# youzhenfei1995/DistributedTF

Measured on AMD Instinct MI355X. Metric: images/sec (whole node) ResNet-56 CIFAR-10 PBT pop=8 at 1/2/4/8 MI355X, higher is better.
Workload: dtype bf16; 1 GPU; model=resnet56_v2_cifar, global_batch=1024, per_member_batch=128, population=8, parallelism=pbt_pop8_8members_per_gpu, backend=hip, exploit_every=25, step_graph=captured

## Files before the change

distributedtf_amd/engine/hip_resnet.py:

```python

from __future__ import annotations

import ctypes
import os
from typing import List, Sequence, Tuple

import torch

from .. import ops
from ..data.datasets import IndexBatch, batch_len
from ..models.resnet import BN_EPS
from .hip_step import (HipBackend, HipPlan, LossRing, PinnedStager, _LIVE_GRAPH_PLANS, _p, advance_steps,
                       graph_state, note_step_advanced, release_graphs, run_captured, run_optimizer, same_batches,
                       upload_hyper)

def _nrep() -> int:
    return ops.build_nrep()


DET_WG_PER_MEMBER = 64
SMALL_POP_MAX = 2
FWD_ITERS_PER_WG = int(os.environ.get("DTF_FWD_ITERS", "4"))
FWD_ITERS_C = {64: 2}
FWD_WG_TARGET = {16: int(os.environ.get("DTF_FWD_WG16", "512"))}
# ... 375 lines not shown
        return p.loss_view()


class _StepPlan(HipPlan):

    def __init__(self, be: HipResNetBackend, slots: List[int], sizes: List[int], src=None, eval_mode=False,
                 elastic_cap=None):
        self.elastic = bool(elastic_cap) and not eval_mode
        self.real_sizes = list(sizes)
        if self.elastic:
            sizes = [int(elastic_cap)] * len(slots)
        self._init_members(be, slots, sizes, eval_mode, counts=self.real_sizes)
        e, dev, N = be.e, be.dev, self.N
        L = be.L
        prog = L.prog
        cfg = L.cfg
        self._wgen, self._elastic_red = [], {}
        self._grab = None
        self._cnt_stage = self._rng_stage = None
        self._stamp_n, self.stamp_rows = {"fwd": 0, "fused": 0}, []
        self._det_rows = self.slab_buf = None
        self._slot_index = {}
        self.uniform = (len(set(sizes)) == 1 and list(slots) == list(range(len(slots))) and not self.elastic
                        and not be.det)
        if self.elastic:
            self.first_t = torch.tensor([self.first[s] for s in slots], dtype=torch.int32, device=dev)
        self.ring = LossRing(len(slots), dev) if (dev.type == "cuda" and not eval_mode and len(slots) <= 1024) else None
        H = cfg.image_size
        self.x_in = torch.zeros(N, H, H, 3, dtype=torch.float32, device=dev)
        self.labels = torch.zeros(N, dtype=torch.int32, device=dev)
        self.xin16 = torch.zeros(N, H, H, 16, dtype=ops.act_dtype(), device=dev)
        self.src = src
        if src is not None:
            self.idx = torch.zeros(N, dtype=torch.long, device=dev)
            self.rng = torch.zeros(2, dtype=torch.int32, device=dev)
        self.v1 = cfg.version == 1
        self.xs, self.hs, self.scs = [], [], []
        self.hb = []
        self.h0 = torch.empty(N, H, H, cfg.num_filters, dtype=ops.act_dtype(), device=dev) if self.v1 else None
        pool = {}

        def act(kind, hw_, c_, i_=0):
            if not self.eval:
                return torch.empty(N, hw_, hw_, c_, dtype=ops.act_dtype(), device=dev)
            key = (kind, hw_, c_, i_ % 2 if kind == "x" else 0)
            if key not in pool:
                pool[key] = torch.empty(N, hw_, hw_, c_, dtype=ops.act_dtype(), device=dev)
            return pool[key]

        hw, c = H, cfg.num_filters
        self.xs.append(act("x", hw, c, 0))
        for bi, blk in enumerate(prog.blocks):
            ca = prog.convs[blk.convs[0]]
            hw_o = hw // blk.stride
            self.hs.append(act("h", hw_o, ca.cout))
            self.scs.append(act("sc", hw_o, ca.cout) if blk.proj is not None else None)
            self.xs.append(act("x", hw_o, ca.cout, bi + 1))
            if self.v1:
                self.hb.append(act("hb", hw_o, ca.cout))
            hw = hw_o
        self._work_cache, self._uniform_geo = {}, {}
        self._pending_slab = None
        if self.eval:
            nb = len(prog.bns)
            cap = e.capacity
            self.ev_stats = torch.zeros(nb, cap, be.nrep, 128, dtype=torch.float32, device=dev)
            self.ev_sink = torch.zeros(cap, be.nrep, 128, dtype=torch.float32, device=dev)
            self.ev_acc = torch.zeros(2, cap, dtype=torch.float32, device=dev)
            self.logits = None
            self._build_eval()
            return
        self.tmp = {}
        hw, c = H, cfg.num_filters
        for st in range(len(cfg.block_sizes)):
            if st > 0:
                hw //= 2
            cc = cfg.num_filters * (2 ** st)
            self.tmp[hw] = dict(g=[torch.empty(N, hw, hw, cc, dtype=ops.act_dtype(), device=dev) for _ in range(2)],
                                dz2=torch.empty(N, hw, hw, cc, dtype=ops.act_dtype(), device=dev),
                                dz1=torch.empty(N, hw, hw, cc, dtype=ops.act_dtype(), device=dev))
        self.pd = {}
        hw = H
        for blk in prog.blocks:
            if blk.proj is not None:
                ci = prog.convs[blk.proj].cin
                self.pd[id(blk)] = torch.empty(N, hw, hw, ci, dtype=ops.act_dtype(), device=dev)
            hw //= blk.stride
        self.dfeat = torch.zeros(N, cfg.final_size, dtype=torch.float32, device=dev)
        v2gpu = dev.type == "cuda" and cfg.version == 2
        self.small_pop = v2gpu and len(slots) <= SMALL_POP_MAX and not be.det
        large = DEFER_MID_CS if (len(slots) <= DEFER_MID_POP and not be.det) else DEFER_LARGE_CS
        self.defer_cs = {16, 32, 64} if self.small_pop else (set(large) if v2gpu else set())
        self._wg_jobs = {}
        self._slab_flip = 0
        self._deferred = []
        self.wslab = dev.type == "cuda"
        self._deferred_dense = []
        self._build()
        assert self._pending_slab is None and not self._deferred and not self._deferred_dense, \
            "every dW slab must be reduced before the optimizer"
        if self.elastic:
            self._work_gen_launch()

    def _work_iters(self, bands, n_wg, det_per=None):
        det = self.be.det
        dper = (det_per or DET_WG_PER_MEMBER) if det else None
        key = ("it", bands, ("det", dper) if det else n_wg)
        w = self._work_cache.get(key)
        if w is None and self.elastic:
            per = dper if det else max(1, n_wg // max(1, len(self.slots)))
            w = self._elastic_table(per, bands, 1)
            self._work_cache[key] = w
        if w is None:
            items = []
            per_member = dper if det else max(1, n_wg // max(1, len(self.slots)))
            for s, n in zip(self.slots, self.sizes):
                total = n * bands
                f = self.first[s] * bands
                chunk = max(1, -(-total // per_member))
                for i in range(0, total, chunk):
                    items.append([f + i, min(chunk, total - i), 0, s])
                if det:
                    items += [[f, 0, 0, s]] * (per_member - -(-total // chunk))
                geo = (-(-total // chunk), chunk, total)
            w = torch.tensor(items, dtype=torch.int32, device=self.be.dev)
            self._work_cache[key] = w
            self._uniform_geo[w.data_ptr()] = geo
        return w

    def _set_uniform(self, a, work):
        if self.uniform:
            a.u_items, a.u_chunk, a.u_per = self._uniform_geo[work.data_ptr()]
            assert a.u_items * len(self.slots) == work.shape[0]

    def _elastic_table(self, per, bands, min_chunk, split=False):
        rows = 2 if split else 1
        host = []
        prop = int(ELASTIC_PROP and not self.be.det)
        layout = elastic_rows([n * bands for n in self.real_sizes], per, min_chunk, prop)
        for (s, n), (r0, nrows, chunk) in zip(zip(self.slots, self.real_sizes), layout):
            total, f = n * bands, self.first[s] * bands
            for j in range(nrows):
                st = j * chunk
                nit = min(chunk, total - st) if st < total else 0
                for z in range(rows):
                    host.append([f + st if nit > 0 else f, nit, z, s])
        assert len(host) == per * len(self.slots) * rows
        w = torch.tensor(host, dtype=torch.int32, device=self.be.dev)
        self._wgen.append((w, per, bands, min_chunk, int(split), prop))
        return w

    def _work_gen_launch(self):
        descs = (WorkGenDesc * len(self._wgen))()
        red = self._elastic_red
        for i, (w, per, bands, mc, sp, prop) in enumerate(self._wgen):
            descs[i] = WorkGenDesc(w.data_ptr(), _p(red.get(w.data_ptr())), per, bands, mc, sp, prop, 0)
        dt = torch.frombuffer(bytearray(bytes(descs)), dtype=torch.uint8).to(self.be.dev)
        self._hold(dt)
        self.launches.insert(0, (ops.lib().dtf_work_gen, (_p(dt), len(self._wgen), _p(self.slots_t),
                                                          _p(self.first_t), len(self.slots), _p(self.cnt))))

    def set_sizes(self, sizes):
        assert self.elastic and len(sizes) == len(self.slots) and max(sizes) <= self.sizes[0]
        if list(sizes) == self.real_sizes:
            return
        self.real_sizes = list(sizes)
        vals = [0.0] * self.e.capacity
# ... 37 lines not shown
        if w is None:
            per_member = max(1, target_items // max(1, len(self.slots)))
            w = self._chunks(lambda n: max(min_chunk, -(-n // per_member)))
            self._work_cache[key] = w
        return w

    def _base_args(self):
        be, e = self.be, self.e
        a = ConvArgs()
        a.img_slot = _p(self.img_slot)
        a.params = _p(e.state)
        a.p_mstride = e.S
        a.cnt = _p(self.cnt)
        a.w_mstride = be.L.wtot
        a.grads = _p(e.grads)
        a.g_mstride = e.Pp
        a.cin_real = 0
        return a

    def _bn(self, idx):
        b = self.be.L.prog.bns[idx]
        return b.gamma_off, b.beta_off

    def _add(self, fn, *args):
        if self._grab is not None:
            self._grab.append((fn, args))
            return
        super()._add(fn, *args)

    def _conv_fwd(self, ci, x, y, stats_bn, in_bn, res=None, proj=None):
        be, L = self.be, self.be.L
        c = L.prog.convs[ci]
        Hi = x.shape[1]
        Ho = Hi // c.stride
        cin = 16 if ci == L.prog.stem else c.cin
        P = (c.k - 1) // 2
        rows = None
        for r in range(min(8, Ho), 0, -1):
            rows_in = (r - 1) * c.stride + c.k
            if Ho % r == 0 and (r * Ho) % 16 == 0 and rows_in * (Hi + 2 * P) * (cin // 8) <= 4 * 256:
                rows = r
                break
        assert rows is not None, ("no valid band for conv", ci)
        s1 = c.k == 3 and c.stride == 1 and cin == c.cout and Hi == 512 // cin and stats_bn is not None
        if s1 and cin == 64 and self.N <= HALF_BANDS_MAX_IMGS and in_bn is not None and not be.det:
            rows = 4
        bands = Ho // rows
        lo = FWD_MIN_WG_SMALL if len(self.slots) <= SMALL_POP_MAX else FWD_MIN_WG
        iters = FWD_ITERS_C.get(cin, FWD_ITERS_PER_WG)
        if cin in FWD_WG_TARGET:
            iters = max(iters, min(8, self.N * bands // FWD_WG_TARGET[cin]))
        n_wg = self._n_wg_iters(self.N * bands, per_wg=iters, lo=lo, hi=max(1024, self.N * bands // iters))
        work = self._work_iters(bands, n_wg)
        a = self._base_args()
        a.x, a.y, a.res = _p(x), _p(y), _p(res)
        a.w, a.w_off = _p(be.wf), L.fwd_off[ci]
        a.work = _p(work)
        if in_bn is not None:
            a.in_gamma, a.in_beta = self._bn(in_bn)
            a.st_in = _p(self._st_r(in_bn))
        if stats_bn is not None:
            a.st_out = _p(self._st_w(stats_bn))
        a.Hi, a.Wi, a.Ho, a.Wo, a.rows = Hi, Hi, Ho, Ho, rows
        if proj is not None:
            cp = L.prog.convs[proj[0]]
            assert (cp.k, cp.stride, cp.cin, cp.cout) == (1, c.stride, c.cin, c.cout) and c.k == 3, (ci, proj[0])
            assert proj[1].shape == y.shape and in_bn is not None and res is None
            a.y2, a.w2_off = _p(proj[1]), L.fwd_off[proj[0]]
        rows_in = (rows - 1) * c.stride + c.k
        tsz = (rows_in * (Hi + 2 * P) * max(_cpad(cin), _cpad_fwd(cin)) + 8 + 63) // 64 * 64
        lds = 1280 + 2 * tsz * 2
        mode = 0 if in_bn is None else 1
        lib = ops.lib()
        if s1 and (rows == 8 or (rows == 4 and cin == 64)):
            self._set_uniform(a, work)
            a.cin_real = self._stamp_row("fwd", "fwd_s1 C=%d in=%d res=%d" % (cin, mode, res is not None))
            lds = 1280 + 2 * ((rows_in * _wpitch(cin) * _cpad_fwd(cin) + 8 + 63) // 64 * 64) * 2
            self._add(lib.dtf_conv_fwd_s1, ctypes.byref(a), cin, mode, int(res is not None), rows, work.shape[0], lds)
        else:
            self._add(lib.dtf_conv_fwd, ctypes.byref(a), cin, c.cout, c.stride, c.k, mode, int(res is not None),
                      int(stats_bn is not None), work.shape[0], lds)
        self._hold(a)

    def _conv_dgrad(self, ci, dy, y, Hi, mode, epi, dy2=None, in_bn=None, res=None, xm=None, ep_bn=None):
        be, L = self.be, self.be.L
        c = L.prog.convs[ci]
        S, K = c.stride, c.k
        Ho = Hi // S
        rows = None
        for r in range(min(8, Hi), 0, -1):
            rows_t = r + K - 1 if S == 1 else (r + K + S - 2) // S + 1
            if Hi % r == 0 and (r * Hi) % 16 == 0 and rows_t * (Ho + 2) * (c.cout // 8) <= 4 * 256:
                rows = r
                break
        assert rows is not None, ("no valid band for dgrad", ci)
        if S == 2 and K == 3:
            assert rows == 8 and Hi == 512 // c.cin, ("stride-2 dgrad geometry", ci, Hi, c.cin, rows)
        rows_t = rows + K - 1 if S == 1 else (rows + K + S - 2) // S + 1
        bands = Hi // rows
        n_wg = self._n_wg_iters(self.N * bands)
        work = self._work_iters(bands, n_wg)
        a = self._base_args()
        a.x, a.x2, a.y, a.res, a.xm = _p(dy), _p(dy2), _p(y), _p(res), _p(xm)
        a.w, a.w_off = _p(be.wd), L.dgr_off[ci]
        a.work = _p(work)
        if in_bn is not None:
            a.in_gamma, a.in_beta = self._bn(in_bn)
            a.st_in, a.st_in_b = _p(be.st_f(in_bn)), _p(be.st_b(in_bn))
        if ep_bn is not None:
            a.ep_gamma, a.ep_beta = self._bn(ep_bn)
            a.st_ep = _p(be.st_f(ep_bn))
            a.st_out = _p(be.st_b(ep_bn))
        a.Hi, a.Wi, a.Ho, a.Wo, a.rows = Hi, Hi, Ho, Ho, rows
        tsz = (rows_t * (Ho + 2) * _cpad(c.cout) + 63) // 64 * 64
        lds = 2304 + 2 * tsz * 2
        lib = ops.lib()
        self._add(lib.dtf_conv_dgrad, ctypes.byref(a), c.cin, c.cout, S, K, mode, epi, work.shape[0], lds)
        self._hold(a)

    @staticmethod
    def _trans_multi(ca_spec):
        return ca_spec.stride == 2 and ca_spec.k == 3 and (ca_spec.cin, ca_spec.cout) in ((16, 32), (32, 64))

    def _add_trans_multi(self, grabbed, ca_spec):
        (f_c, args_c), (f_a, args_a), (f_b, args_b) = grabbed
        lib = ops.lib()
        assert [ops.launcher_name(f) for f in (f_c, f_a, f_b)] == ["dtf_conv_wgrad", "dtf_conv_dgrad", "dtf_conv_wgrad"]
        assert args_c[1:6] == (ca_spec.cin, ca_spec.cout, 2, 3, 1) and args_c[6] == 2
        assert args_a[1:7] == (ca_spec.cin, ca_spec.cout, 2, 1, 0, 0)
        assert args_b[1:7] == (ca_spec.cin, ca_spec.cout, 2, 1, 1, 0)
        ac, aa, ab = args_c[0]._obj, args_a[0]._obj, args_b[0]._obj
        ac.n_main, aa.n_main, ab.n_main = args_c[7], args_a[7], args_b[7]
        nblocks = args_c[7] + args_a[7] + args_b[7]
        lds = max(args_c[8], args_a[8], args_b[8])
        self._add(lib.dtf_conv_trans_multi, ctypes.byref(ac), ctypes.byref(aa), ctypes.byref(ab), ca_spec.cin,
                  ca_spec.cout, nblocks, lds)

    def _conv_wgrad(self, ci, x, dy, mode_x, mode_dy, x_bn=None, dy_bn=None, dy2=None, cin_real=None):
        be, L, e = self.be, self.be.L, self.e
        c = L.prog.convs[ci]
        Hi = x.shape[1]
        Ho = Hi // c.stride
        cin = 16 if ci == L.prog.stem else c.cin
        P = (c.k - 1) // 2
        rows = None
        for r in range(min(8, Ho), 0, -1):
            if Ho % r or (r * Ho) % 32:
                continue
            rows_in = (r - 1) * c.stride + c.k
            if rows_in * (Hi + 2 * P) * (cin // 8) <= 4 * 256 and r * Ho * (c.cout // 8) <= 2 * 256:
                rows = r
                break
        if rows is None:
            rows = _pick_rows(Ho, Ho, 1, 32, target_items=1, max_rows=8)
        wn = c.cout * c.k * c.k * c.cin
        n_wg = max(64, min(WGRAD_WG_PER_MEMBER * len(self.slots), int(12e6 / (4.0 * wn))))
        if self.be.det and not self.wslab:
            n_wg = len(self.slots)
        work = self._work_iters(Ho // rows, n_wg)
        a = self._base_args()
        a.x, a.dy, a.dy2 = _p(x), _p(dy), _p(dy2)
        a.work = _p(work)
        a.g_off = c.off
        a.cin_real = c.cin if cin_real is None else cin_real
        if x_bn is not None:
            a.x_gamma, a.x_beta = self._bn(x_bn)
            a.st_x = _p(be.st_f(x_bn))
        if dy_bn is not None:
            a.in_gamma, a.in_beta = self._bn(dy_bn)
            a.st_in, a.st_in_b = _p(be.st_f(dy_bn)), _p(be.st_b(dy_bn))
        a.Hi, a.Wi, a.Ho, a.Wo, a.rows = Hi, Hi, Ho, Ho, rows
        rows_in = (rows - 1) * c.stride + c.k
        assert 32 % Ho == 0, "wgrad k-step addressing needs Wo | 32"
        xt = (rows_in * (Hi + 2 * P) * _cpad(cin) + 63) // 64 * 64
        dt = (rows * Ho * _cpad(c.cout) + 63) // 64 * 64
        lds = 1536 + 2 * (xt + dt) * 2
        lib = ops.lib()
        if self.wslab:
            kel = c.cout * c.k * c.k * a.cin_real
            a.slab = _p(self._layer_slab(work.shape[0] * kel))
            self._deferred_dense.append((a.slab, self._slab_table(work), c.off, kel))
        self._add(lib.dtf_conv_wgrad, ctypes.byref(a), cin, c.cout, c.stride, c.k, mode_x, mode_dy, work.shape[0], lds)
        self._hold(a)

    def _conv_bwd_fused(self, ci, dy, dz_out, x, mode_dy, dy2=None, dy_bn=None, x_bn=None, res=None, ident_x=False,
                        dy3=None, dy_out=None, chain_bn=None, chain_h=None):
        be, L = self.be, self.be.L
        c = L.prog.convs[ci]
        assert c.stride == 1 and c.k == 3 and c.cin == c.cout
        assert (mode_dy == 3) == (dy3 is not None)
        C, H = c.cin, x.shape[1]
        rows = None
        for r in (8, 4, 2):
            if H % r == 0 and (r * H) % 32 == 0 and (r + 2) * (H + 2) * (C // 8) <= 4 * 256:
                rows = r
                break
        assert rows == 8 and H == 512 // C and x.shape[2] == H, (C, H, rows)
        for t in (dy, dy2, dy3, dy_out, dz_out, x, res):
            assert t is None or tuple(t.shape) == (self.N, H, H, C), (t.shape, C, H)
        bands = H // rows
        if C in self.defer_cs:
            assert chain_bn is None, "chain_bn needs the fused launch (the deferred path is v2-only)"
            return self._conv_bwd_deferred(ci, rows, dy, dz_out, x, mode_dy, dy2, dy_bn, x_bn, res, ident_x, dy3,
                                           dy_out)
        n_wg = self._fused_nwg(C, bands, mode_dy)
        work = self._work_iters(bands, n_wg)
        a = self._bwd_args(ci, work, rows, dy, dy2, dy3, x, dy_bn, None if ident_x else x_bn,
                           dgrad=(dz_out, res, dy_out))
        if chain_bn is not None:
            assert ident_x and mode_dy == 2 and tuple(chain_h.shape) == (self.N, H, H, C)
            a.x3 = _p(chain_h)
            a.ep_gamma, a.ep_beta = self._bn(chain_bn)
            a.st_ep = _p(self._st_r(chain_bn))
            a.st_out = _p(be.st_b(chain_bn))
        tsz = ((rows + 2) * _wpitch(C) * _cpad(C) + 8 + 63) // 64 * 64
        raw = C >= 64
        nbuf = 4
        lds = 2304 + (nbuf * tsz + (2 * rows * H * _cpad(C) if raw else 0)) * 2
        if C == 16 and _lib_knob("dtf_fused16_wlds"):
# ... 231 lines not shown
        if self.eval:
            self._add(lib.dtf_bn_eval_stats, _p(e.state), e.S, 3 * e.Pp, _p(be.bn_table_t), len(L.bn_table),
                      _p(self.ev_stats), be.stats_bn_stride, _p(self.slots_t), nslots, _p(self.cnt))
        if self.src is not None:
            self._add("augment", None)
        else:
            self._add(lib.dtf_prep_input, _p(self.x_in), _p(self.xin16), self.N * L.cfg.image_size ** 2, 3)

    def _step_epilogue(self):
        be, e, L = self.be, self.e, self.be.L
        self._flush_slab()
        self._flush_deferred()
        self._add(ops.lib().dtf_bn_step_end, _p(e.state), e.S, 3 * e.Pp, _p(be.bn_table_t), len(L.bn_table),
                  _p(be.stats[0]), _p(be.stats[1]), be.stats_bn_stride, _p(self.slots_t), len(self.slots),
                  _p(self.cnt), _p(e.grads), e.Pp)
        self._add("optim", None)
        self._add("step", None)

    def _head_args(self, train):
        be, e, L = self.be, self.e, self.be.L
        prog, cfg = L.prog, L.cfg
        hwork = self._head_work() if train else self._work_member(target_items=HEAD_ITEMS)
        ha = self._hold(HeadArgs())
        ha.x, ha.labels, ha.work = _p(self.xs[-1]), _p(self.labels), _p(hwork)
        ha.params, ha.p_mstride = _p(e.state), e.S
        ha.gamma_off, ha.beta_off = (-1, -1) if self.v1 else self._bn(prog.final_bn)
        ha.dw_off, ha.db_off = prog.dense_w_off, prog.dense_b_off
        ha.g_mstride, ha.cnt = e.Pp, _p(self.cnt)
        ha.hw, ha.C, ha.ncls, ha.train = L.final_hw, cfg.final_size, cfg.num_classes, int(train)
        if train:
            st = (be.stats, be.stats) if self.v1 else (be.st_f(prog.final_bn), be.st_b(prog.final_bn))
            ha.st_f, ha.st_b, ha.grads = _p(st[0]), _p(st[1]), _p(e.grads)
            ha.dfeat, ha.loss, ha.correct = _p(self.dfeat), _p(be.loss), _p(be.correct)
            ha.loss_scale = be.loss_scale
            ha.scale_tab = _p(e.lscale) if e.dynamic_loss_scale else None
            self._head_slab(ha, hwork)
        else:
            ha.st_f = _p(self.ev_sink if self.v1 else self._st_r(prog.final_bn))
            ha.st_b, ha.correct, ha.loss = _p(self.ev_sink), _p(self.ev_acc[0]), _p(self.ev_acc[1])
            ha.loss_scale = 1.0
        self._add(ops.lib().dtf_head, ctypes.byref(ha), hwork.shape[0])
        return ha

    def _build(self):
        if self.v1:
            return self._build_v1()
        be, e, L = self.be, self.e, self.be.L
        prog, cfg = L.prog, L.cfg
        lib = ops.lib()
        N = self.N
        self._step_prologue()
        self._forward_v2()
        nblk = len(prog.blocks)
        fb = prog.final_bn
        hw = L.final_hw
        ha = self._head_args(True)
        hwL = self.xs[-1].shape[1]
        g_cur = self.tmp[hwL]["g"][0]
        self._add(lib.dtf_head_bwd_apply, _p(self.xs[-1]), _p(self.dfeat), _p(g_cur), _p(self.img_slot), _p(e.state),
                  e.S, ha.gamma_off, ha.beta_off, _p(be.st_f(fb)), _p(be.st_b(fb)), _p(self.cnt), hw,
                  cfg.final_size, N)
        pend = None
        stem_dy = None
        for i in range(nblk - 1, -1, -1):
            blk = prog.blocks[i]
            bn1, bn2 = blk.bns
            x, h = self.xs[i], self.hs[i]
            Hi, Ho = x.shape[1], h.shape[1]
            T = self.tmp[Ho]
            if h.shape[3] in self.defer_cs:
                T = dict(T, dz2=self._fresh_like(T["dz2"]))
            ca, cb = blk.convs
            if pend is not None:
                dz1p, xp, addp, outp, bn1p = pend
                self._conv_bwd_fused(cb, dz1p, T["dz2"], h, mode_dy=3 if addp is not None else 2, dy2=xp,
                                     dy3=addp, dy_out=outp, dy_bn=bn1p, x_bn=bn2)
                g_cur, pend = outp, None
            else:
                self._conv_bwd_fused(cb, g_cur, T["dz2"], h, mode_dy=0, x_bn=bn2)
            Tin = self.tmp[Hi] if Hi != Ho else T
            pd = None
            ca_spec = prog.convs[ca]
            if blk.proj is not None and self._trans_multi(ca_spec):
                pd = self.pd[id(blk)]
                self._grab = []
                self._conv_wgrad(ca, x, T["dz2"], mode_x=1, mode_dy=2, x_bn=bn1, dy_bn=bn2, dy2=h)
                self._conv_dgrad(blk.proj, g_cur, pd, Hi, mode=0, epi=0)
                self._conv_wgrad(blk.proj, x, g_cur, mode_x=1, mode_dy=0, x_bn=bn1)
                grabbed, self._grab = self._grab, None
                self._add_trans_multi(grabbed, ca_spec)
                self._conv_dgrad(ca, T["dz2"], Tin["dz1"], Hi, mode=2, epi=2 | 1, dy2=h, in_bn=bn2, res=pd, xm=x,
                                 ep_bn=bn1)
            elif blk.proj is not None:
                pd = self.pd[id(blk)]
                self._conv_dgrad(blk.proj, g_cur, pd, Hi, mode=0, epi=0)
                self._conv_wgrad(blk.proj, x, g_cur, mode_x=1, mode_dy=0, x_bn=bn1)
            if blk.proj is not None and self._trans_multi(ca_spec):
                pass
            elif ca_spec.stride == 1 and ca_spec.cin == ca_spec.cout:
                self._conv_bwd_fused(ca, T["dz2"], Tin["dz1"], x, mode_dy=2, dy2=h, dy_bn=bn2, x_bn=bn1, res=pd)
            else:
                self._conv_dgrad(ca, T["dz2"], Tin["dz1"], Hi, mode=2, epi=2 | (1 if pd is not None else 0), dy2=h,
                                 in_bn=bn2, res=pd, xm=x, ep_bn=bn1)
                self._conv_wgrad(ca, x, T["dz2"], mode_x=1, mode_dy=2, x_bn=bn1, dy_bn=bn2, dy2=h)
            add = None if blk.proj is not None else g_cur
            if i == 0 and add is None:
                stem_dy = (Tin["dz1"], x, bn1)
                break
            g_next = Tin["g"][1] if g_cur is Tin["g"][0] else Tin["g"][0]
            if x.shape[3] in self.defer_cs:
                g_next = self._fresh_like(Tin["g"][0])
            if i > 0:
                pend = (Tin["dz1"], x, add, g_next, bn1)
            else:
                self._bn_bwd_apply(Tin["dz1"], x, add, g_next, bn1)
            g_cur = g_next
        if stem_dy is not None:
            dz1, x0, bn1 = stem_dy
            self._conv_wgrad(prog.stem, self.xin16, dz1, mode_x=0, mode_dy=2, dy_bn=bn1, dy2=x0,
                             cin_real=cfg.in_channels)
        else:
            self._conv_wgrad(prog.stem, self.xin16, g_cur, mode_x=0, mode_dy=0, cin_real=cfg.in_channels)
        self._emit_deferred_wgrad()
        self._step_epilogue()

    def _forward_v2(self):
        prog = self.be.L.prog
        first_bn = prog.blocks[0].bns[0]
        self._conv_fwd(prog.stem, self.xin16, self.xs[0], stats_bn=first_bn, in_bn=None)
        nblk = len(prog.blocks)
        for i, blk in enumerate(prog.blocks):
            bn1, bn2 = blk.bns
            nxt = prog.blocks[i + 1].bns[0] if i + 1 < nblk else prog.final_bn
            x, h, y = self.xs[i], self.hs[i], self.xs[i + 1]
            self._conv_fwd(blk.convs[0], x, h, stats_bn=bn2, in_bn=bn1,
                           proj=(blk.proj, self.scs[i]) if blk.proj is not None else None)
            res = self.scs[i] if blk.proj is not None else x
            self._conv_fwd(blk.convs[1], h, y, stats_bn=nxt, in_bn=bn2, res=res)

    def _forward_v1(self):
        prog, cfg = self.be.L.prog, self.be.L.cfg
        lib = ops.lib()
        H = cfg.image_size
        self._conv_fwd(prog.stem, self.xin16, self.h0, stats_bn=prog.stem_bn, in_bn=None)
        self._bn_ew(lib.dtf_bn_add_relu, (H * H, cfg.num_filters), prog.stem_bn, self.h0, out=self.xs[0])
        for i, blk in enumerate(prog.blocks):
            bna, bnb = blk.bns
            x, ha, hb, y = self.xs[i], self.hs[i], self.hb[i], self.xs[i + 1]
            if blk.proj is not None:
                self._conv_fwd(blk.proj, x, self.scs[i], stats_bn=blk.proj_bn, in_bn=None)
            self._conv_fwd(blk.convs[0], x, ha, stats_bn=bna, in_bn=None)
            self._conv_fwd(blk.convs[1], ha, hb, stats_bn=bnb, in_bn=bna)
            hw_o = y.shape[1] * y.shape[2]
            if blk.proj is not None:
                self._bn_ew(lib.dtf_bn_add_relu, (hw_o, y.shape[3]), bnb, hb, bn2=blk.proj_bn, h2=self.scs[i], out=y)
            else:
                self._bn_ew(lib.dtf_bn_add_relu, (hw_o, y.shape[3]), bnb, hb, add=x, out=y)

    def _st_r(self, bn):
        return self.ev_stats[bn] if self.eval else self.be.st_f(bn)

    def _st_w(self, bn):
        return self.ev_sink if self.eval else self.be.st_f(bn)

    def _build_eval(self):
        self._step_prologue()
        if self.v1:
            self._forward_v1()
        else:
            self._forward_v2()
        self.head_args = self._head_args(False)

    def want_logits(self):
        if self.logits is None:
            self.logits = torch.zeros(self.N, self.be.L.cfg.num_classes, dtype=torch.float32, device=self.be.dev)
# ... 125 lines not shown
```

distributedtf_amd/ops/csrc/conv.hip:

```cpp
#include "common.h"

#define BN_EPS 1e-5f
#ifndef DTF_FUSED_SB16
#define DTF_FUSED_SB16 0
#endif
#ifndef DTF_FUSED16_WLDS
#define DTF_FUSED16_WLDS 1
#endif
#ifndef DTF_TRANSFORM8_PK
#define DTF_TRANSFORM8_PK 1
#endif
#ifndef DTF_BWD_COEFREG
#define DTF_BWD_COEFREG 1
#endif
#ifndef DTF_FWD_COEFREG
#define DTF_FWD_COEFREG 1
#endif
#ifndef DTF_COEF_SPLIT
#define DTF_COEF_SPLIT 1
#endif
#ifndef DTF_COEF_W0
#define DTF_COEF_W0 1
#endif
#ifndef DTF_FUSED16_M3_WAVES
// ... 1048 lines not shown
  for (int k = 0; k < nit; ++k) {
    const int it = it0 + k;
    const int img = it / BANDS, r0 = (it % BANDS) * ROWS;
    const bool more = k + 1 < nit;
    const long band = (long)img * IMG + r0 * ROW;
    uint2 rres[MT];
    if constexpr (RESID) {
#pragma unroll
      for (int i = 0; i < MT; ++i) rres[i] = nres[i];
    }
    if (more) {
      const int nimg = (it + 1) / BANDS;
      tgy0 = ((it + 1) % BANDS) * ROWS - 1;
      st.template load<LMODE>(tv, unused, a.x + nimg * IMG, nullptr, tgy0);
      if constexpr (RESID) {
        const long nband = (long)nimg * IMG + ((it + 1) % BANDS) * ROWS * ROW;
#pragma unroll
        for (int i = 0; i < MT; ++i) nres[i] = *reinterpret_cast<const uint2*>(a.res + nband + pofs[i]);
      }
    }
    const bf16_t* tile = SBUF(k);
#pragma unroll
    for (int i = 0; i < MT; ++i) {
      f32x4_t acc = {0.f, 0.f, 0.f, 0.f};
      [[maybe_unused]] f32x4_t pa;
#pragma unroll
      for (int s = 0; s < KS; ++s) {
        const bf16x8_t b = *reinterpret_cast<const bf16x8_t*>(tile + tbo[i] + tapoff[s]);
        acc = mfma16(afr[s], b, acc);
        if constexpr (PROJ) {
          if (s == 4 * C / 32) pa = mfma16(pfr, b, (f32x4_t){0.f, 0.f, 0.f, 0.f});
        }
      }
      f32x2_t v0 = {acc[0], acc[1]}, v1 = {acc[2], acc[3]};
      if constexpr (RESID) {
        v0 += unpk2(rres[i].x);
        v1 += unpk2(rres[i].y);
      }
      uint2 pk;
      pk.x = pk2(v0);
      pk.y = pk2(v1);
      st_act8(a.y + band + pofs[i], pk);
      if constexpr (PROJ) {
        uint2 pp;
        pp.x = pk2((f32x2_t){pa[0], pa[1]});
        pp.y = pk2((f32x2_t){pa[2], pa[3]});
        st_act8(a.y2 + band + pofs[i], pp);
      }
      const f32x2_t r0v = unpk2(pk.x), r1v = unpk2(pk.y);
      ssum[0] += r0v;
      ssum[1] += r1v;
      ssq[0] += r0v * r0v;
      ssq[1] += r1v * r1v;
    }
    if (more) {
      if constexpr (CREG)
        st.store1r(SBUF(k + 1), tv, tgy0, csc, csh);
      else
        st.template store<LMODE>(SBUF(k + 1), tv, unused, tgy0, coef);
    }
    __syncthreads();
  }
#undef SBUF
  STAMP(3);
  const float s4[4] = {ssum[0].x, ssum[0].y, ssum[1].x, ssum[1].y};
  const float q4[4] = {ssq[0].x, ssq[0].y, ssq[1].x, ssq[1].y};
  reduce_stats_to_lds(acc_lds, s4, q4, co0, lane);
  __syncthreads();
  flush_stats_r(a.st_out, acc_lds, slot, C, bid);
  STAMP_DRAIN(4);
  STAMP_FLUSH(a.cin_real, nit);
}

template <int C, int MODE_IN, bool RESID, int ROWS = 8, bool PROJ = false>
__global__ __launch_bounds__(256) void conv_fwd_s1_kernel(ConvArgs a) {
  extern __shared__ __attribute__((aligned(16))) char smem[];
  conv_fwd_s1_body<C, MODE_IN, RESID, ROWS, PROJ>(a, (int)blockIdx.x, smem);
}


template <int CI, int CO, int S, int K, int MODE_IN, int EPI>
__device__ __forceinline__ void conv_dgrad_body(const ConvArgs& a, const int bid, char* smem) {
  constexpr bool MASK = (EPI & 6) != 0, IDENT = (EPI & 4) != 0, STATS = (EPI & 2) != 0 && !IDENT;
  constexpr int NT = CI / 16;
  constexpr int WPT = 4 / NT;
  constexpr int KTOT = K * K * CO;
  constexpr int KS = (KTOT + 31) / 32;
  constexpr int P = (K - 1) / 2;
  float* coef = reinterpret_cast<float*>(smem);
  float* ecoef = coef + 192;
  float* acc_lds = ecoef + 256;
  bf16_t* tile0 = reinterpret_cast<bf16_t*>(smem + 2304);

  const int4 wk = a.work[bid];
  DTF_WG_CHECK(wk.x >= 0 && wk.y >= 0 && wk.w >= 0 && wk.z >= 0 && a.Hi > 0 && a.Wi > 0 && a.rows > 0);
  const int it0 = wk.x, nit = wk.y, slot = wk.w;
  const int wave = threadIdx.x >> 6, lane = threadIdx.x & 63;
  make_coef<CO, MODE_IN>(coef, a, slot, a.cnt[slot] * (float)(a.Ho * a.Wo), a.st_in, a.st_in_b, a.in_gamma, a.in_beta);
  if constexpr (MASK) {
    const int c = threadIdx.x;
    if (c < CI) {
      const float* prow = a.params + (long)slot * a.p_mstride;
      float scale = 1.f, shift = 0.f, mean = 0.f, inv = 1.f;
      if constexpr (!IDENT)
        bn_fwd_coef(stats_row(a.st_ep, slot), a.cnt[slot] * (float)(a.Hi * a.Wi), prow[a.ep_gamma + c],
                    prow[a.ep_beta + c], c, scale, shift, mean, inv);
      ecoef[c] = scale;
      ecoef[64 + c] = shift;
      ecoef[128 + c] = mean;
      ecoef[192 + c] = inv;
    }
    if (threadIdx.x < 128) acc_lds[threadIdx.x] = 0.f;
  }
  const int ct = wave % NT;
  bf16x8_t afr[KS];
  {
    const bf16_t* wb = a.w + (long)slot * a.w_mstride + a.w_off + (long)(ct * 16 + (lane & 15)) * KTOT;
#pragma unroll
    for (int s = 0; s < KS; ++s) {
      const int k0 = 32 * s + 8 * (lane >> 4);
      bf16x8_t v = {0, 0, 0, 0, 0, 0, 0, 0};
      if (k0 < KTOT) v = *reinterpret_cast<const bf16x8_t*>(wb + k0);
      afr[s] = v;
    }
  }
  const int rows = a.rows;
  const int bands = a.Hi / rows;
  auto dy_lo = [&](int iy0) {
    const int lo_num = iy0 + P - K + 1;
    return lo_num >= 0 ? lo_num / S : -((-lo_num + S - 1) / S);
  };
  const int rows_t = (S == 1) ? rows + K - 1 : (rows + K + S - 2) / S + 1;
  const int wp = a.Wo + 2;
  const int tsz = (rows_t * wp * cpad<CO>() + 63) & ~63;
#define TILEBUF(i) (tile0 + ((i) & 1) * tsz)
  const int ntiles = rows * a.Wi / 16;
  const long img_elems = (long)a.Ho * a.Wo * CO;
  constexpr bool PAR = S == 2 && K == 3 && (512 / CI) * 8 / 16 == 4 * WPT;
  constexpr int WI = 512 / CI;
  if constexpr (PAR) DTF_WG_CHECK(a.Wi == WI && rows == 8 && MAXT == 4);
  auto par_pix = [&](int i, int iy0_, int& iy_, int& ix_) {
    const int q = (wave / NT) * 16 + (lane & 15), cy = q / (WI / 2), cx = q % (WI / 2);
    iy_ = iy0_ + 2 * cy + (i >> 1);
    ix_ = 2 * cx + (i & 1);
  };
  int tapoff[KS];
#pragma unroll
  for (int s = 0; s < KS; ++s) {
    const int k0 = 32 * s + 8 * (lane >> 4);
    const int tap = k0 / CO, c0 = k0 % CO;
    tapoff[s] = -((tap / K) * wp + (tap % K)) * cpad<CO>() + c0;
  }
  float ssum[4] = {0.f, 0.f, 0.f, 0.f}, ssq[4] = {0.f, 0.f, 0.f, 0.f};
  TileRegs<CO, MODE_IN, 4> rg;
  TileDesc<CO, 4> td;
  tile_desc_init<CO, 4>(td, rows_t, -1, wp, a.Wo);
  __syncthreads();
  {
    const int img = it0 / bands, iy0 = (it0 % bands) * rows;
    const bf16_t* x2 = a.x2 ? a.x2 + img * img_elems : nullptr;
    tile_load<CO, MODE_IN, 4>(rg, td, a.x + img * img_elems, x2, dy_lo(iy0), a.Ho, a.Wo);
    tile_store<CO, MODE_IN, 4>(TILEBUF(0), rg, td, a.x + img * img_elems, x2, dy_lo(iy0), a.Ho, a.Wo, coef);
  }
  __syncthreads();
  for (int k = 0; k < nit; ++k) {
    const int it = it0 + k;
    const int img = it / bands, iy0 = (it % bands) * rows;
    const int oy_lo = dy_lo(iy0);
    const bool more = k + 1 < nit;
    const int nimg_ = (it + 1) / bands, niy0 = ((it + 1) % bands) * rows;
    const bf16_t* nx2 = a.x2 ? a.x2 + nimg_ * img_elems : nullptr;
    uint2 rres[MAXT], xres[MAXT];
#pragma unroll
    for (int i = 0; i < MAXT; ++i) {
      int py_, px_;
      if constexpr (PAR) {
        par_pix(i, iy0, py_, px_);
      } else {
        const int t = min(wave / NT + WPT * i, ntiles - 1);
        const int p = t * 16 + (lane & 15);
        py_ = iy0 + p / a.Wi;
        px_ = p % a.Wi;
      }
      const long o = (((long)img * a.Hi + py_) * a.Wi + px_) * CI + ct * 16 + (lane >> 4) * 4;
      if constexpr (EPI & 1) rres[i] = *reinterpret_cast<const uint2*>(a.res + o);
      if constexpr (MASK) xres[i] = *reinterpret_cast<const uint2*>(a.xm + o);
    }
    if (more) tile_load<CO, MODE_IN, 4>(rg, td, a.x + nimg_ * img_elems, nx2, dy_lo(niy0), a.Ho, a.Wo);
    const bf16_t* tile = TILEBUF(k);
#pragma unroll
    for (int i = 0; i < MAXT; ++i) {
      const int t = wave / NT + WPT * i;
      if (t >= ntiles) break;
      f32x4_t acc = {0.f, 0.f, 0.f, 0.f};
      int iy, ix;
      if constexpr (PAR) {
        par_pix(i, iy0, iy, ix);
      } else {
        const int p = t * 16 + (lane & 15);
        iy = iy0 + p / a.Wi;
        ix = p % a.Wi;
      }
      const int ci0 = ct * 16 + (lane >> 4) * 4;
      const long o = (((long)img * a.Hi + iy) * a.Wi + ix) * CI + ci0;
      uint2 rr = make_uint2(0, 0), xr = make_uint2(0, 0);
      if constexpr (EPI & 1) rr = rres[i];
      if constexpr (MASK) xr = xres[i];
      const bf16_t* tb = tile + ((iy + P - oy_lo) * wp + ix + P + 1) * cpad<CO>();
      if constexpr (PAR) {
        constexpr int CJ = CO / 32;
#pragma unroll
        for (int ay = 0; ay < ((i >> 1) ? 2 : 1); ++ay) {
          const int ky = (i >> 1) ? 2 * ay : 1;
#pragma unroll
          for (int ax = 0; ax < ((i & 1) ? 2 : 1); ++ax) {
            const int kx = (i & 1) ? 2 * ax : 1;
            const bf16_t* tp = tile + ((((iy + 1 - ky) >> 1) - oy_lo) * wp + ((ix + 1 - kx) >> 1) + 1) * cpad<CO>() +
                               8 * (lane >> 4);
#pragma unroll
            for (int j = 0; j < CJ; ++j)
              acc = mfma16(afr[(ky * 3 + kx) * CJ + j], *reinterpret_cast<const bf16x8_t*>(tp + 32 * j), acc);
          }
        }
      } else {
#pragma unroll
      for (int s = 0; s < KS; ++s) {
        const int k0 = 32 * s + 8 * (lane >> 4);
        bf16x8_t b = {0, 0, 0, 0, 0, 0, 0, 0};
        if constexpr (S == 1) {
          if (k0 < KTOT) b = *reinterpret_cast<const bf16x8_t*>(tb + tapoff[s]);
        } else if (k0 < KTOT) {
          const int tap = k0 / CO, c0 = k0 % CO;
          const int ky = tap / K, kx = tap % K;
          const int ty = iy + P - ky, tx = ix + P - kx;
          bool ok = true;
          int oy = ty, ox = tx;
          if constexpr (S > 1) {
            ok = (ty >= 0) && (tx >= 0) && (ty % S == 0) && (tx % S == 0);
            oy = ty / S;
            ox = tx / S;
          }
          const int lr = oy - oy_lo, lc = ox + 1;
          if (ok && lr >= 0 && lr < rows_t && lc >= 0 && lc < wp)
            b = *reinterpret_cast<const bf16x8_t*>(tile + lds_off<CO>(lr, lc, wp, c0 >> 3));
        }
        acc = mfma16(afr[s], b, acc);
      }
      }
      float v[4] = {acc[0], acc[1], acc[2], acc[3]};
      if constexpr (EPI & 1) {
        v[0] += bf2f((bf16_t)(rr.x & 0xffff));
        v[1] += bf2f((bf16_t)(rr.x >> 16));
        v[2] += bf2f((bf16_t)(rr.y & 0xffff));
        v[3] += bf2f((bf16_t)(rr.y >> 16));
      }
      float xv[4] = {0.f, 0.f, 0.f, 0.f};
      if constexpr (MASK) {
        xv[0] = bf2f((bf16_t)(xr.x & 0xffff));
        xv[1] = bf2f((bf16_t)(xr.x >> 16));
        xv[2] = bf2f((bf16_t)(xr.y & 0xffff));
        xv[3] = bf2f((bf16_t)(xr.y >> 16));
#pragma unroll
        for (int r = 0; r < 4; ++r) {
          const int c = ci0 + r;
          const float pre = xv[r] * ecoef[c] + ecoef[64 + c];
          v[r] = pre > 0.f ? v[r] : 0.f;
        }
      }
      uint2 pk;
      pk.x = pack2bf(v[0], v[1]);
      pk.y = pack2bf(v[2], v[3]);
      st_act8(a.y + o, pk);
      if constexpr (STATS) {
        const float dz[4] = {bf2f((bf16_t)(pk.x & 0xffff)), bf2f((bf16_t)(pk.x >> 16)), bf2f((bf16_t)(pk.y & 0xffff)),
                             bf2f((bf16_t)(pk.y >> 16))};
#pragma unroll
        for (int r = 0; r < 4; ++r) {
          const int c = ci0 + r;
          ssum[r] += dz[r];
          ssq[r] += dz[r] * (xv[r] - ecoef[128 + c]) * ecoef[192 + c];
        }
      }
    }
    if (more)
      tile_store<CO, MODE_IN, 4>(TILEBUF(k + 1), rg, td, a.x + nimg_ * img_elems, nx2, dy_lo(niy0), a.Ho, a.Wo,
                                 coef);
    __syncthreads();
  }
  if constexpr (STATS) {
    reduce_stats_to_lds(acc_lds, ssum, ssq, ct * 16 + (lane >> 4) * 4, lane);
    __syncthreads();
    flush_stats_r(a.st_out, acc_lds, slot, CI, bid);
  }
}


typedef short s16x4_t __attribute__((ext_vector_type(4)));

__device__ __forceinline__ s16x4_t ds_read_tr(const bf16_t* p) {
  return __builtin_amdgcn_ds_read_tr16_b64_v4i16((__attribute__((address_space(3))) s16x4_t*)(p));
}

template <int CI, int CO, int S, int K, int MODE_IN, int EPI>
__global__ __launch_bounds__(256) void conv_dgrad_kernel(ConvArgs a) {
// ... 810 lines not shown
  return DTF_CHECK_LAUNCH();
}

DTF_DEBUG_EXPORT(conv)

DTF_API int dtf_stamp_read(void* dst, long bytes) {
#if DTF_STAMP
  if (bytes > (long)sizeof(dtf_stamps)) bytes = (long)sizeof(dtf_stamps);
  return (int)hipMemcpyFromSymbol(dst, HIP_SYMBOL(dtf_stamps), bytes);
#else
  (void)dst;
  (void)bytes;
  return -1;
#endif
}

DTF_API int dtf_conv_args_size() { return (int)sizeof(ConvArgs); }

DTF_API int dtf_conv_trans_multi(const ConvArgs* c, const ConvArgs* a, const ConvArgs* b, int ci, int co, int nblocks,
                                 int lds, hipStream_t stream) {
  DTF_HOST_CHECK(c->work != nullptr && a->work != nullptr && b->work != nullptr);
  DTF_HOST_CHECK(nblocks == c->n_main + a->n_main + b->n_main && lds <= 160 * 1024);
  if (nblocks <= 0) return 0;
#define TM_CASE(CI_, CO_)                                                                                   \
  if (ci == CI_ && co == CO_) {                                                                           \
    hipLaunchKernelGGL((conv_trans_multi_kernel<CI_, CO_>), dim3(nblocks), dim3(256), lds, stream, *c, *a, *b); \
    return DTF_CHECK_LAUNCH();                                                                            \
  }
  TM_CASE(16, 32)
  TM_CASE(32, 64)
#undef TM_CASE
  return -1;
}
DTF_API int dtf_fused16_wlds() { return DTF_FUSED16_WLDS; }
DTF_API int dtf_fused16_m3_waves() { return DTF_FUSED16_M3_WAVES; }
DTF_API int dtf_fused16_m2_waves() { return DTF_FUSED16_M2_WAVES; }

DTF_API int dtf_cpad_fwd(int c) { return c == 16 ? cpad_fwd<16>() : c == 32 ? cpad_fwd<32>() : c == 64 ? cpad_fwd<64>() : -1; }
DTF_API int dtf_wpitch(int c) { return c == 16 ? wpitch<16>() : c == 32 ? wpitch<32>() : c == 64 ? wpitch<64>() : -1; }

DTF_API int dtf_conv_fwd(const ConvArgs* args, int cin, int cout, int s, int k, int mode, int resid, int stats,
                         int nblocks, int lds, hipStream_t stream) {
  if (args->y2 != nullptr) {
    if (!(k == 3 && s == 2 && mode == 1 && resid == 0 && stats == 1 && DTF_ALIGNED16(args->y2))) return -1;
    if (cin == 16 && cout == 32)
      return launch(conv_fwd_kernel<16, 32, 2, 3, 1, false, true, true>, nblocks, lds, stream, *args);
    if (cin == 32 && cout == 64)
      return launch(conv_fwd_kernel<32, 64, 2, 3, 1, false, true, true>, nblocks, lds, stream, *args);
    return -1;
  }
  FWD_CASE(16, 16, 1, 3, 0, false, true)
  FWD_CASE(16, 16, 1, 3, 1, false, true)
  FWD_CASE(16, 16, 1, 3, 1, true, true)
  FWD_CASE(32, 32, 1, 3, 1, false, true)
  FWD_CASE(32, 32, 1, 3, 1, true, true)
  FWD_CASE(64, 64, 1, 3, 1, false, true)
  FWD_CASE(64, 64, 1, 3, 1, true, true)
  FWD_CASE(16, 32, 2, 3, 1, false, true)
  FWD_CASE(32, 64, 2, 3, 1, false, true)
  FWD_CASE(16, 16, 1, 1, 1, false, false)
  FWD_CASE(16, 32, 2, 1, 1, false, false)
  FWD_CASE(32, 64, 2, 1, 1, false, false)
  FWD_CASE(16, 32, 2, 3, 0, false, true)
  FWD_CASE(32, 64, 2, 3, 0, false, true)
  FWD_CASE(16, 16, 1, 1, 0, false, true)
  FWD_CASE(16, 32, 2, 1, 0, false, true)
  FWD_CASE(32, 64, 2, 1, 0, false, true)
  FWD_CASE(32, 32, 1, 3, 0, false, true)
  FWD_CASE(64, 64, 1, 3, 0, false, true)
  return -1;
}

DTF_API int dtf_conv_dgrad(const ConvArgs* args, int cin, int cout, int s, int k, int mode, int epi, int nblocks,
                           int lds, hipStream_t stream) {
  DGRAD_CASE(16, 16, 1, 3, 0, 2)
  DGRAD_CASE(32, 32, 1, 3, 0, 2)
  DGRAD_CASE(64, 64, 1, 3, 0, 2)
  DGRAD_CASE(16, 16, 1, 3, 2, 2)
  DGRAD_CASE(32, 32, 1, 3, 2, 2)
  DGRAD_CASE(64, 64, 1, 3, 2, 2)
  DGRAD_CASE(16, 16, 1, 3, 2, 3)
  DGRAD_CASE(16, 32, 2, 3, 2, 3)
  DGRAD_CASE(32, 64, 2, 3, 2, 3)
  DGRAD_CASE(16, 16, 1, 1, 0, 0)
  DGRAD_CASE(16, 32, 2, 1, 0, 0)
  DGRAD_CASE(32, 64, 2, 1, 0, 0)
  DGRAD_CASE(16, 16, 1, 1, 2, 0)
  DGRAD_CASE(16, 32, 2, 1, 2, 0)
  DGRAD_CASE(32, 64, 2, 1, 2, 0)
  DGRAD_CASE(16, 32, 2, 3, 2, 5)
  DGRAD_CASE(32, 64, 2, 3, 2, 5)
  DGRAD_CASE(16, 16, 1, 3, 2, 5)
  DGRAD_CASE(16, 16, 1, 3, 2, 4)
  DGRAD_CASE(32, 32, 1, 3, 2, 4)
  DGRAD_CASE(64, 64, 1, 3, 2, 4)
  return -1;
}

#define FUSED_CASE(CC, M, E)                                                                          \
  if (c == CC && mode_dy == M && epi == E)                                                           \
    return launch(conv_bwd_fused_kernel<CC, M, E>, nblocks, lds, stream, *args);

DTF_API int dtf_conv_bwd_fused(const ConvArgs* args, int c, int mode_dy, int epi, int nblocks, int lds,
                               hipStream_t stream) {
  if (nblocks <= 0) return 0;
  DTF_HOST_CHECK(args->n_main > 0 && nblocks >= args->n_main && args->rows == 8);
  if (nblocks > args->n_main) {
    DTF_HOST_CHECK(args->rslab != nullptr && args->rtab != nullptr && args->grads != nullptr);
    DTF_HOST_CHECK(args->r_c == 16 || args->r_c == 32 || args->r_c == 64);
    DTF_HOST_CHECK(args->r_nblk > 0 && (nblocks - args->n_main) % args->r_nblk == 0);
  }
  FUSED_CASE(16, 0, 0)
  FUSED_CASE(32, 0, 0)
  FUSED_CASE(64, 0, 0)
  FUSED_CASE(16, 3, 0)
  FUSED_CASE(32, 3, 0)
  FUSED_CASE(64, 3, 0)
  FUSED_CASE(16, 2, 0)
  FUSED_CASE(32, 2, 0)
  FUSED_CASE(64, 2, 0)
  FUSED_CASE(16, 2, 1)
  FUSED_CASE(16, 2, 3)
  FUSED_CASE(32, 2, 3)
  FUSED_CASE(64, 2, 3)
  FUSED_CASE(16, 2, 11)
  FUSED_CASE(32, 2, 11)
  FUSED_CASE(64, 2, 11)
  return -1;
}

DTF_API int dtf_conv_bwd_dg(const ConvArgs* a, int c, int mode_dy, int epi, int rows, int nblocks, int lds,
                            hipStream_t stream) {
  if (nblocks <= 0) return 0;
  DTF_HOST_CHECK(lds <= 160 * 1024);
  DTF_HOST_CHECK(a->work != nullptr && nblocks == a->n_main && a->rows == rows);
  if (rows == 4) {
#define DG4_CASE(CC, M)                                                                                      \
    if (c == CC && mode_dy == M && epi == 0) {                                                              \
      hipLaunchKernelGGL((conv_bwd_dg_kernel<CC, M, 0, 4>), dim3(nblocks), dim3(256), lds, stream, *a);     \
      return DTF_CHECK_LAUNCH();                                                                            \
    }
    DG4_CASE(64, 0) DG4_CASE(64, 2) DG4_CASE(64, 3)
#undef DG4_CASE
    return -1;
  }
#define DG_CASE(CC, M, E)                                                                                    \
  if (c == CC && mode_dy == M && epi == E) {                                                                \
    hipLaunchKernelGGL((conv_bwd_dg_kernel<CC, M, E>), dim3(nblocks), dim3(256), lds, stream, *a);          \
    return DTF_CHECK_LAUNCH();                                                                              \
  }
  DG_CASE(16, 0, 0) DG_CASE(32, 0, 0) DG_CASE(64, 0, 0)
  DG_CASE(16, 3, 0) DG_CASE(32, 3, 0) DG_CASE(64, 3, 0)
  DG_CASE(16, 2, 0) DG_CASE(32, 2, 0) DG_CASE(64, 2, 0)
  DG_CASE(16, 2, 1)
#undef DG_CASE
  return -1;
}

DTF_API int dtf_conv_wgrad_all(const void* jobs, const void* map, int nblocks, int cset, int lds, hipStream_t stream) {
  if (nblocks <= 0) return 0;
  DTF_HOST_CHECK(jobs != nullptr && map != nullptr && lds <= 160 * 1024 && (cset == 0 || cset == 1));
  if (cset == 0)
    hipLaunchKernelGGL((conv_wgrad_all_kernel<64, 32>), dim3(nblocks), dim3(256), lds, stream,
                       reinterpret_cast<const ConvArgs*>(jobs), reinterpret_cast<const int4*>(map));
  else
    hipLaunchKernelGGL((conv_wgrad_all_kernel<16, 16>), dim3(nblocks), dim3(256), lds, stream,
// ... 29 lines not shown
```

Baseline: 359,800 images/s.

## Fuse 1x1 stride-2 projection dgrad into the 3x3 stride-2 dgrad kernel

For v2 downsampling blocks, the projection shortcut's data gradient (1x1 stride-2 conv) is no longer computed as a separate dgrad into a scratch buffer and then added back as a residual. It is accumulated directly inside the parity-class tiles of the 3x3 stride-2 dgrad via extra MFMAs on the even-pixel class. The trans_multi launch drops its dgrad sub-job, and the pd scratch buffers are no longer allocated for these blocks. This removes one kernel's work plus a full write and read of the projection gradient tensor. In exchange the main dgrad kernel carries extra registers and loads, which may affect occupancy.

After: 362,700 images/s (median of 6 runs). No clear change (+0.8%).

```diff
diff --git a/distributedtf_amd/engine/hip_resnet.py b/distributedtf_amd/engine/hip_resnet.py
--- a/distributedtf_amd/engine/hip_resnet.py
+++ b/distributedtf_amd/engine/hip_resnet.py
@@ -481,7 +481,7 @@
         self.pd = {}
         hw = H
         for blk in prog.blocks:
-            if blk.proj is not None:
+            if blk.proj is not None and (self.v1 or not self._trans_multi(prog.convs[blk.convs[0]])):
                 ci = prog.convs[blk.proj].cin
                 self.pd[id(blk)] = torch.empty(N, hw, hw, ci, dtype=ops.act_dtype(), device=dev)
             hw //= blk.stride
@@ -685,7 +685,7 @@
                       int(stats_bn is not None), work.shape[0], lds)
         self._hold(a)
 
-    def _conv_dgrad(self, ci, dy, y, Hi, mode, epi, dy2=None, in_bn=None, res=None, xm=None, ep_bn=None):
+    def _conv_dgrad(self, ci, dy, y, Hi, mode, epi, dy2=None, in_bn=None, res=None, xm=None, ep_bn=None, proj=None):
         be, L = self.be, self.be.L
         c = L.prog.convs[ci]
         S, K = c.stride, c.k
@@ -715,6 +715,11 @@
             a.st_ep = _p(be.st_f(ep_bn))
             a.st_out = _p(be.st_b(ep_bn))
         a.Hi, a.Wi, a.Ho, a.Wo, a.rows = Hi, Hi, Ho, Ho, rows
+        if proj is not None:
+            cp = L.prog.convs[proj[0]]
+            assert (cp.k, cp.stride, cp.cin, cp.cout) == (1, 2, c.cin, c.cout) and (S, K) == (2, 3), (ci, proj[0])
+            assert proj[1].shape == dy.shape and res is None and epi & 16
+            a.x3, a.w2_off = _p(proj[1]), L.dgr_off[proj[0]]
         tsz = (rows_t * (Ho + 2) * _cpad(c.cout) + 63) // 64 * 64
         lds = 2304 + 2 * tsz * 2
         lib = ops.lib()
@@ -726,18 +731,18 @@
         return ca_spec.stride == 2 and ca_spec.k == 3 and (ca_spec.cin, ca_spec.cout) in ((16, 32), (32, 64))
 
     def _add_trans_multi(self, grabbed, ca_spec):
-        (f_c, args_c), (f_a, args_a), (f_b, args_b) = grabbed
+        (f_c, args_c), (f_b, args_b) = grabbed
         lib = ops.lib()
-        assert [ops.launcher_name(f) for f in (f_c, f_a, f_b)] == ["dtf_conv_wgrad", "dtf_conv_dgrad", "dtf_conv_wgrad"]
+        assert [ops.launcher_name(f) for f in (f_c, f_b)] == ["dtf_conv_wgrad", "dtf_conv_wgrad"]
         assert args_c[1:6] == (ca_spec.cin, ca_spec.cout, 2, 3, 1) and args_c[6] == 2
-        assert args_a[1:7] == (ca_spec.cin, ca_spec.cout, 2, 1, 0, 0)
         assert args_b[1:7] == (ca_spec.cin, ca_spec.cout, 2, 1, 1, 0)
-        ac, aa, ab = args_c[0]._obj, args_a[0]._obj, args_b[0]._obj
-        ac.n_main, aa.n_main, ab.n_main = args_c[7], args_a[7], args_b[7]
-        nblocks = args_c[7] + args_a[7] + args_b[7]
-        lds = max(args_c[8], args_a[8], args_b[8])
+        ac, ab = args_c[0]._obj, args_b[0]._obj
+        aa = self._base_args()
+        aa.work = ac.work
+        ac.n_main, aa.n_main, ab.n_main = args_c[7], 0, args_b[7]
         self._add(lib.dtf_conv_trans_multi, ctypes.byref(ac), ctypes.byref(aa), ctypes.byref(ab), ca_spec.cin,
-                  ca_spec.cout, nblocks, lds)
+                  ca_spec.cout, args_c[7] + args_b[7], max(args_c[8], args_b[8]))
+        self._hold(aa)
 
     def _conv_wgrad(self, ci, x, dy, mode_x, mode_dy, x_bn=None, dy_bn=None, dy2=None, cin_real=None):
         be, L, e = self.be, self.be.L, self.e
@@ -1135,15 +1140,13 @@
             pd = None
             ca_spec = prog.convs[ca]
             if blk.proj is not None and self._trans_multi(ca_spec):
-                pd = self.pd[id(blk)]
                 self._grab = []
                 self._conv_wgrad(ca, x, T["dz2"], mode_x=1, mode_dy=2, x_bn=bn1, dy_bn=bn2, dy2=h)
-                self._conv_dgrad(blk.proj, g_cur, pd, Hi, mode=0, epi=0)
                 self._conv_wgrad(blk.proj, x, g_cur, mode_x=1, mode_dy=0, x_bn=bn1)
                 grabbed, self._grab = self._grab, None
                 self._add_trans_multi(grabbed, ca_spec)
-                self._conv_dgrad(ca, T["dz2"], Tin["dz1"], Hi, mode=2, epi=2 | 1, dy2=h, in_bn=bn2, res=pd, xm=x,
-                                 ep_bn=bn1)
+                self._conv_dgrad(ca, T["dz2"], Tin["dz1"], Hi, mode=2, epi=2 | 16, dy2=h, in_bn=bn2, xm=x, ep_bn=bn1,
+                                 proj=(blk.proj, g_cur))
             elif blk.proj is not None:
                 pd = self.pd[id(blk)]
                 self._conv_dgrad(blk.proj, g_cur, pd, Hi, mode=0, epi=0)
diff --git a/distributedtf_amd/ops/csrc/conv.hip b/distributedtf_amd/ops/csrc/conv.hip
--- a/distributedtf_amd/ops/csrc/conv.hip
+++ b/distributedtf_amd/ops/csrc/conv.hip
@@ -1154,6 +1154,9 @@
 template <int CI, int CO, int S, int K, int MODE_IN, int EPI>
 __device__ __forceinline__ void conv_dgrad_body(const ConvArgs& a, const int bid, char* smem) {
   constexpr bool MASK = (EPI & 6) != 0, IDENT = (EPI & 4) != 0, STATS = (EPI & 2) != 0 && !IDENT;
+  constexpr bool PROJ = (EPI & 16) != 0;
+  static_assert(!PROJ || (S == 2 && K == 3 && CO % 32 == 0 && !(EPI & 1)), "projection: class 0 of the PAR path");
+  constexpr int PJ = PROJ ? CO / 32 : 1;
   constexpr int NT = CI / 16;
   constexpr int WPT = 4 / NT;
   constexpr int KTOT = K * K * CO;
@@ -1196,6 +1199,14 @@
       afr[s] = v;
     }
   }
+  [[maybe_unused]] bf16x8_t pfr[PJ];
+  if constexpr (PROJ) {
+    DTF_WG_CHECK(a.x3 != nullptr);
+    const bf16_t* wb = a.w + (long)slot * a.w_mstride + a.w2_off + (long)(ct * 16 + (lane & 15)) * CO +
+                       8 * (lane >> 4);
+#pragma unroll
+    for (int j = 0; j < PJ; ++j) pfr[j] = *reinterpret_cast<const bf16x8_t*>(wb + 32 * j);
+  }
   const int rows = a.rows;
   const int bands = a.Hi / rows;
   auto dy_lo = [&](int iy0) {
@@ -1210,6 +1221,7 @@
   const long img_elems = (long)a.Ho * a.Wo * CO;
   constexpr bool PAR = S == 2 && K == 3 && (512 / CI) * 8 / 16 == 4 * WPT;
   constexpr int WI = 512 / CI;
+  static_assert(!PROJ || PAR, "projection: parity-class tiles only");
   if constexpr (PAR) DTF_WG_CHECK(a.Wi == WI && rows == 8 && MAXT == 4);
   auto par_pix = [&](int i, int iy0_, int& iy_, int& ix_) {
     const int q = (wave / NT) * 16 + (lane & 15), cy = q / (WI / 2), cx = q % (WI / 2);
@@ -1257,6 +1269,14 @@
       const long o = (((long)img * a.Hi + py_) * a.Wi + px_) * CI + ct * 16 + (lane >> 4) * 4;
       if constexpr (EPI & 1) rres[i] = *reinterpret_cast<const uint2*>(a.res + o);
       if constexpr (MASK) xres[i] = *reinterpret_cast<const uint2*>(a.xm + o);
+    }
+    [[maybe_unused]] bf16x8_t gfr[PJ];
+    if constexpr (PROJ) {
+      int py_, px_;
+      par_pix(0, iy0, py_, px_);
+      const bf16_t* gp = a.x3 + img * img_elems + ((long)(py_ >> 1) * a.Wo + (px_ >> 1)) * CO + 8 * (lane >> 4);
+#pragma unroll
+      for (int j = 0; j < PJ; ++j) gfr[j] = *reinterpret_cast<const bf16x8_t*>(gp + 32 * j);
     }
     if (more) tile_load<CO, MODE_IN, 4>(rg, td, a.x + nimg_ * img_elems, nx2, dy_lo(niy0), a.Ho, a.Wo);
     const bf16_t* tile = TILEBUF(k);
@@ -1292,6 +1312,12 @@
 #pragma unroll
             for (int j = 0; j < CJ; ++j)
               acc = mfma16(afr[(ky * 3 + kx) * CJ + j], *reinterpret_cast<const bf16x8_t*>(tp + 32 * j), acc);
+          }
+        }
+        if constexpr (PROJ) {
+          if (i == 0) {
+#pragma unroll
+            for (int j = 0; j < PJ; ++j) acc = mfma16(pfr[j], gfr[j], acc);
           }
         }
       } else {
@@ -2268,6 +2294,11 @@
   DGRAD_CASE(16, 16, 1, 3, 2, 3)
   DGRAD_CASE(16, 32, 2, 3, 2, 3)
   DGRAD_CASE(32, 64, 2, 3, 2, 3)
+  DGRAD_CASE(16, 32, 2, 3, 2, 2)
+  DGRAD_CASE(32, 64, 2, 3, 2, 2)
+  if ((epi & 16) && !(args->x3 != nullptr && DTF_ALIGNED16(args->x3) && args->w2_off % 8 == 0)) return -1;
+  DGRAD_CASE(16, 32, 2, 3, 2, 18)
+  DGRAD_CASE(32, 64, 2, 3, 2, 18)
   DGRAD_CASE(16, 16, 1, 1, 0, 0)
   DGRAD_CASE(16, 32, 2, 1, 0, 0)
   DGRAD_CASE(32, 64, 2, 1, 0, 0)
```
